# privacy-scaling-explorations/zkevm-specs

Hardware: AMD Instinct MI355X
Metric: BN254 constraint-rows/sec (higher is better)
Workload: dtype u256 (BN254 Fr: 4xu64 canonical cells, u32-limb Montgomery); 1 GPU; EVM circuit, 2^18 execution steps per GPU, mixed-opcode synthetic trace (BASELINE configs[2]); RW table 816377 rows, bytecode table 43913 rows; steps_per_gpu=262144, rw_rows=816377, bytecode_rows=43913, witness_copies=3

## Files before the change

### zkevm_specs_amd/csrc/zkevm_hip.hip

```cpp
#include <hip/hip_runtime.h>
#include <hip/hip_ext.h>
#include <stdio.h>
#include <string.h>
#include <stdlib.h>
#include <chrono>
#include <string>
#include <vector>

#include <atomic>
#include <mutex>
#include <dlfcn.h>

#include "../../include/zkevm_hip.h"
#include "kernels.hpp"
#include "dist_tally.hpp"
#include "host_index.hpp"
#include "code_dir_build.hpp"

#define ZK_MAX_DEVICES 64
#define ZK_ECDSA_CHUNK_LANES (1ull << 17)
static std::mutex g_dev_mutex;
static hipStream_t g_own_stream[ZK_MAX_DEVICES] = {nullptr};
static hipStream_t g_batch_stream[ZK_MAX_DEVICES][2] = {{nullptr}};
static hipStream_t g_side_stream[ZK_MAX_DEVICES] = {nullptr};
// ... 69 lines not shown
    return 0;
}
extern "C" void zk_shutdown(void) {
    arena_release_all();
    std::lock_guard<std::mutex> lock(g_dev_mutex);
    for (int d = 0; d < ZK_MAX_DEVICES; d++)
        if (g_own_stream[d]) {
            if (hipSetDevice(d) == hipSuccess) {
                (void)hipStreamDestroy(g_own_stream[d]);
                if (g_zero_row[d]) (void)hipFree(g_zero_row[d]);
                if (g_secp_comb[d]) (void)hipFree(g_secp_comb[d]);
                g_secp_comb[d] = nullptr;
            }
            for (int k = 0; k < 2; k++) {
                if (g_batch_stream[d][k]) (void)hipStreamDestroy(g_batch_stream[d][k]);
                g_batch_stream[d][k] = nullptr;
            }
            if (g_side_stream[d]) (void)hipStreamDestroy(g_side_stream[d]);
            g_side_stream[d] = nullptr;
            for (int k = 0; k < 4; k++) {
                if (g_block_stream[d][k]) (void)hipStreamDestroy(g_block_stream[d][k]);
                g_block_stream[d][k] = nullptr;
            }
            g_own_stream[d] = nullptr;
            g_zero_row[d] = nullptr;
        }
    t_stream = nullptr;
    t_device = -1;
}
extern "C" int zk_set_stream(void* st) {
    ARG_TRY(t_device >= 0, "zk_set_stream: call zk_init first");
    t_stream = st ? (hipStream_t)st : g_own_stream[t_device];
    return 0;
}
struct zk_session;
static int session_rebind_stream(zk_session* s, hipStream_t st);
extern "C" int zk_session_set_stream(zk_session* s, void* st) {
    ARG_TRY(s, "zk_session_set_stream: null session");
    return session_rebind_stream(s, (hipStream_t)st);
}

__global__ void tally_reset_kernel(ZkTally* t, u32* counter = nullptr) {
    t[threadIdx.x].fail_count = 0ull;
    t[threadIdx.x].first_fail = ~0ull;
    if (counter && threadIdx.x == 0) *counter = 0u;
}


__global__ void slots_fill_kernel(u32* slots, u32 n) {
    u32 i = blockIdx.x * blockDim.x + threadIdx.x;
    if (i < n) slots[i] = ZK_EMPTY_SLOT;
}

template <u64 (*HASH)(const ZkTable&, u32)>
__global__ void index_build_kernel(ZkTable t, u32* slots, const ZkRwMeta* unless_dense = nullptr) {
    u32 r = blockIdx.x * blockDim.x + threadIdx.x;
    if (r >= t.n || (unless_dense && unless_dense->dense)) return;
    u32 s = (u32)HASH(t, r) & t.mask;
    while (atomicCAS(&slots[s], ZK_EMPTY_SLOT, r) != ZK_EMPTY_SLOT) s = (s + 1) & t.mask;
}
__global__ void slots_fill_unless_dense_kernel(u32* slots, u32 n, const ZkRwMeta* unless_dense) {
    u32 i = blockIdx.x * blockDim.x + threadIdx.x;
    if (i < n && !unless_dense->dense) slots[i] = ZK_EMPTY_SLOT;
}
__global__ void mpt_index_build_kernel(ZkTable t, u32* slots) {
    u32 r = blockIdx.x * blockDim.x + threadIdx.x;
    if (r >= t.n) return;
    const u64 h = state_mpt_key_hash(t, r);
    u32 s = (u32)h & t.mask;
    const u32 v = state_mpt_slot_value(t, r, h);
    while (atomicCAS(&slots[s], ZK_EMPTY_SLOT, v) != ZK_EMPTY_SLOT) s = (s + 1) & t.mask;
}
__global__ void rw_dense_check_kernel(ZkTable t, ZkRwMeta* meta) {
    const u32 r = blockIdx.x * blockDim.x + threadIdx.x;
    if (r >= t.n) return;
    const u64* p = t.cells + (u64)r * RW_NCELLS * 4;
    const u64* p0 = t.cells;
    const u64 base = p0[0];
    const bool ok = (p0[1] | p0[2] | p0[3]) == 0 && (p[1] | p[2] | p[3]) == 0 && p[0] == base + r && base + r >= base;
    if (r == 0) meta->base = base;
    if (!ok) atomicAnd(&meta->dense, 0u);
}

struct EvmSortArgs {
    const u64* steps;
    u32 n_pairs;
    u32* hist;
    u32* hist_next;
    u32* taken;
    uint16_t* bin16;
    u32* group_start;
    u32* perm;
    ZkTally* tally;
    u32* defer_count;
    u32* early_host;
    u32 early_seq;
};
#define EVM_EARLY_WORD 36u
__device__ __forceinline__ void evm_state_hist_body(u32 vblock, const u64* steps, u32 n_pairs, u32* hist, u32* taken, uint16_t* bin16, ZkTally* tally,
                                                    u32* defer_count) {
    __shared__ u32 local[EVM_N_BINS];
    if (vblock == 0) {
        if (threadIdx.x == 0 && defer_count) *defer_count = 0u;
        if (threadIdx.x == 0) {
            tally->fail_count = 0ull;
            tally->first_fail = ~0ull;
        }
        for (u32 k = threadIdx.x; k < EVM_N_BINS; k += blockDim.x) taken[k] = 0;
    }
    for (u32 k = threadIdx.x; k < EVM_N_BINS; k += blockDim.x) local[k] = 0;
    __syncthreads();
    u32 i = vblock * blockDim.x + threadIdx.x;
    if (i < n_pairs) {
        const u32 bin = evm_state_bin((u32)steps[((u64)i * STEP_NCELLS + S_STATE) * 4]);
        bin16[i] = (uint16_t)bin;
        atomicAdd(&local[bin], 1u);
    }
    __syncthreads();
    for (u32 k = threadIdx.x; k < EVM_N_BINS; k += blockDim.x)
        if (local[k]) atomicAdd(&hist[k], local[k]);
}
__global__ void evm_state_hist_kernel(const u64* steps, u32 n_pairs, u32* hist, u32* taken, uint16_t* bin16, ZkTally* tally, u32* defer_count) {
    evm_state_hist_body(blockIdx.x, steps, n_pairs, hist, taken, bin16, tally, defer_count);
}
__device__ __forceinline__ void evm_state_scatter_body(u32 vblock, const uint16_t* bin16, u32 n_pairs, const u32* hist, u32* hist_next,
                                                       u32* taken, u32* group_start, u32* perm, u32* early_host = nullptr, u32 early_seq = 0u) {
    __shared__ u32 sa[EVM_N_BINS], sb[EVM_N_BINS];
    __shared__ u32 local[EVM_N_BINS];
    __shared__ u32 base[EVM_N_BINS];
    __shared__ u32 gsh[EVM_N_GROUPS + 1];
    const u32 k = threadIdx.x;
    u32 c = 0, c_real = 0;
    if (k < EVM_N_BINS) {
        c_real = hist[k];
        c = k < (u32)EVM_GROUP_WARM * 128u ? ((c_real + 63u) & ~63u) : c_real;
        sa[k] = c;
        local[k] = 0;
        if (vblock == 0) hist_next[k] = 0;
    }
    __syncthreads();
    u32* src = sa;
    u32* dst = sb;
    for (u32 off = 1; off < EVM_N_BINS; off <<= 1) {
        if (k < EVM_N_BINS) dst[k] = src[k] + (k >= off ? src[k - off] : 0u);
        __syncthreads();
        u32* t = src; src = dst; dst = t;
    }
    u32 excl = 0;
    if (k < EVM_N_BINS) {
        excl = src[k] - c;
        if (vblock == 0) {
            if ((k & 127u) == 0) group_start[k >> 7] = gsh[k >> 7] = excl;
            if (k == EVM_N_BINS - 1) group_start[EVM_N_GROUPS] = gsh[EVM_N_GROUPS] = src[k];
            for (u32 j = c_real; j < c; j++) perm[excl + j] = EVM_NO_PAIR;
        }
    }
    const u32 i = vblock * blockDim.x + threadIdx.x;
    u32 bin = 0, rank = 0;
    if (i < n_pairs) {
        bin = bin16[i];
        rank = atomicAdd(&local[bin], 1u);
    }
    __syncthreads();
    if (vblock == 0 && k == 0 && early_host) {
        __hip_atomic_store(&early_host[EVM_EARLY_WORD], gsh[EVM_GROUP_WARM + 1] - gsh[EVM_GROUP_WARM], __ATOMIC_RELAXED, __HIP_MEMORY_SCOPE_SYSTEM);
        __hip_atomic_store(&early_host[EVM_EARLY_WORD + 1], gsh[EVM_GROUP_COLD + 1] - gsh[EVM_GROUP_COLD], __ATOMIC_RELAXED, __HIP_MEMORY_SCOPE_SYSTEM);
        __threadfence_system();
        __hip_atomic_store(&early_host[EVM_EARLY_WORD + 2], early_seq, __ATOMIC_RELEASE, __HIP_MEMORY_SCOPE_SYSTEM);
    }
    if (k < EVM_N_BINS && local[k]) base[k] = excl + atomicAdd(&taken[k], local[k]);
    __syncthreads();
    if (i < n_pairs) perm[base[bin] + rank] = i;
}
__global__ __launch_bounds__(1024) void evm_state_scatter_kernel(const uint16_t* bin16, u32 n_pairs, const u32* hist, u32* hist_next,
                                                                 u32* taken, u32* group_start, u32* perm) {
    evm_state_scatter_body(blockIdx.x, bin16, n_pairs, hist, hist_next, taken, group_start, perm);
}
__global__ __launch_bounds__(256) void evm_open_fill_kernel(uint4* ff, u64 n_ff, uint4* zero, u64 n_zero) {
    const u64 stride = (u64)gridDim.x * blockDim.x;
    const uint4 F = make_uint4(~0u, ~0u, ~0u, ~0u), Z = make_uint4(0u, 0u, 0u, 0u);
    for (u64 i = (u64)blockIdx.x * blockDim.x + threadIdx.x; i < n_ff; i += stride) ff[i] = F;
    for (u64 i = (u64)blockIdx.x * blockDim.x + threadIdx.x; i < n_zero; i += stride) zero[i] = Z;
}
__device__ __forceinline__ void rw_prepare_quad(const ZkTable& t, u64* keys, EvmDyn* dyn, u32 vthread) {
    const u32 r = vthread >> 2, q = vthread & 3u;
    const bool in = r < t.n;
    uint4 c0 = make_uint4(0, 0, 0, 0), c1 = c0, c2 = c0;
    u64 base = 0;
    u32 flags = 3u;
    if (in) {
        const uint4* p = reinterpret_cast<const uint4*>(t.cells + (u64)r * RW_NCELLS * 4) + q;
        c0 = p[0];
        c1 = p[4];
        c2 = p[8];
        if (q == 0) {
            base = t.cells[0];
            if (t.flags) flags = t.flags[r];
        }
    }
    bool fit, dense_ok;
    u64 w0 = 0, w1 = 0, w2 = 0, w3 = 0;
    const bool z0hi = (c0.y | c0.z | c0.w) == 0u, z1hi = (c1.y | c1.z | c1.w) == 0u, z2hi = (c2.y | c2.z | c2.w) == 0u;
    const bool z0 = z0hi && c0.x == 0u, z1 = z1hi && c1.x == 0u, z2 = z2hi && c2.x == 0u;
    if (q == 0) {
        const u64 rwc = (u64)c0.x | ((u64)c0.y << 32);
        dense_ok = (c0.z | c0.w) == 0u && rwc == base + r && base + r >= base;
        fit = z1hi && c1.x <= 255u;
        w0 = (u64)(c1.x & 0xffu) << 8 | ((u64)(flags & 3u) << 56) | (1ull << 63);
        w2 = (u64)c2.x | ((u64)c2.y << 32);
        w3 = (u64)c2.z | ((u64)c2.w << 32);
    } else if (q == 1) {
        dense_ok = z0;
        fit = z1 && z2hi;
        w0 = (u64)c2.x << 24;
    } else if (q == 2) {
        dense_ok = true;
        fit = z0hi && c0.x <= 255u && (c1.z | c1.w) == 0u && z2hi && c2.x <= 255u;
        w0 = (u64)(c0.x & 0xffu) | ((u64)(c2.x & 0xffu) << 16);
        w1 = (u64)c1.x | ((u64)c1.y << 32);
    } else {
        dense_ok = true;
        fit = z0 && z1 && z2;
    }
    const u32 qshift = threadIdx.x & 60u;
    const bool fits = ((__ballot(fit) >> qshift) & 0xfull) == 0xfull;
    const unsigned long long nd = __ballot(in && !dense_ok);
    if (nd != 0ull && (threadIdx.x & 63u) == 0) atomicOr(&dyn->rw_sparse, 1u);
    if (r == 0 && q == 0 && in) dyn->rw_base = base;
#pragma unroll
    for (int m = 1; m <= 2; m <<= 1) {
        w0 |= __shfl_xor(w0, m);
        w1 |= __shfl_xor(w1, m);
        w2 |= __shfl_xor(w2, m);
        w3 |= __shfl_xor(w3, m);
    }
    if (!fits) w0 = w1 = w2 = w3 = 0;
    if (in && q < 2) {
        const u64 a = q == 0 ? w0 : w2, b2 = q == 0 ? w1 : w3;
        reinterpret_cast<uint4*>(keys + (u64)r * 4)[q] = make_uint4((u32)a, (u32)(a >> 32), (u32)b2, (u32)(b2 >> 32));
    }
}
#define EVM_OPEN_TABLES 8
struct EvmOpenTables {
    ZkTable t[EVM_OPEN_TABLES];
    u32 block_start[EVM_OPEN_TABLES + 2];
    const u64* wds;
    u32 n_wds;
    EvmDyn* dyn;
    ZkTally* tally;
    ZkTable rw;
    u64* rw_keys;
    u32 dir_block0, rw_block0;
    DirBuild dir;
    const u64* steps;
    u32 n_steps;
    u32* step_recs;
    u32 rec_block0;
    EvmSortArgs sort;
    u32 hist_block0;
    u32 lat_period;
#ifdef ZK_DIAG_P1
    u32 diag_skip;
#endif
};
__device__ __forceinline__ void evm_open_small_tables(const EvmOpenTables& o, u32 block) {
    int k = 0;
#pragma unroll
    for (int j = 1; j <= EVM_OPEN_TABLES; j++) k += block >= o.block_start[j] ? 1 : 0;
    const u32 r = (block - o.block_start[k]) * blockDim.x + threadIdx.x;
    if (k == EVM_OPEN_TABLES) {
        const bool nz = r < o.n_wds && !fr_is_zero(fr_load(o.wds + ((u64)r * 4 + 3) * 4));
        const unsigned long long b = __ballot(nz);
        if (b && (threadIdx.x & 63u) == 0) atomicAdd(&o.dyn->agg_total_wds, (u32)__popcll(b));
        return;
    }
    const ZkTable& t = o.t[k];
    const bool in = r < t.n;
    if (k == 0) {
        bool caller = false, present = false, invalid = false, bad = false;
        if (in) {
            const Fr tag = zk_table_cell(t, r, 1), lo = zk_table_cell(t, r, 3), hi = zk_table_cell(t, r, 4);
            caller = fr_eq_u64(tag, 4);
            present = caller && !(fr_is_zero(lo) && fr_is_zero(hi));
            const bool inv_row = fr_eq_u64(tag, 10);
            bad = inv_row && t.flags && (t.flags[r] & 1u);
            invalid = inv_row && fr_eq_u64(lo, 1);
        }
        const unsigned long long bc = __ballot(caller), bp = __ballot(present), bi = __ballot(invalid), bb = __ballot(bad);
        if ((threadIdx.x & 63u) == 0) {
            if (bc) atomicAdd(&o.dyn->agg_max_txs, (u32)__popcll(bc));
            if (bp) atomicAdd(&o.dyn->agg_total_txs, (u32)__popcll(bp));
            if (bi) atomicAdd(&o.dyn->agg_invalid_txs, (u32)__popcll(bi));
            if (bb) atomicOr(&o.dyn->agg_bad_invalid_rows, 1u);
        }
    }
    if (!in) return;
    u64 h;
    switch (k) {
    case 0: h = tx_key_hash(t, r); break;
    case 1: h = blk_key_hash(t, r); break;
    case 2: h = bc_key_hash(t, r); break;
    case 3: h = copy_key_hash(t, r); break;
    case 4: h = keccak_key_hash(t, r); break;
    case 5: h = expt_key_hash(t, r); break;
    case 6: h = sig_key_hash(t, r); break;
    default: h = ecc_key_hash(t, r); break;
    }
    u32* slots = const_cast<u32*>(t.slots);
    u32 s = (u32)h & t.mask;
    while (atomicCAS(&slots[s], ZK_EMPTY_SLOT, r) != ZK_EMPTY_SLOT) s = (s + 1) & t.mask;
}
__global__ __launch_bounds__(256) void evm_open_phase1_kernel(EvmOpenTables o) {
    if (blockIdx.x == 0 && threadIdx.x < 2) {
        o.tally[threadIdx.x].fail_count = 0ull;
        o.tally[threadIdx.x].first_fail = ~0ull;
    }
    u32 b = blockIdx.x;
    if (o.lat_period > 1u && b < o.rec_block0) {
        const u32 q = b / o.lat_period;
        b = (b == q * o.lat_period && q < o.rw_block0) ? q : o.rw_block0 + b - (q + 1u < o.rw_block0 ? q + 1u : o.rw_block0);
    }
#ifdef ZK_DIAG_P1
    {
        const u32 range = b < o.dir_block0 ? 1u : b < o.hist_block0 ? 2u : b < o.rw_block0 ? 4u : b < o.rec_block0 ? 8u : 16u;
        if (o.diag_skip & range) return;
    }
#endif
    if (b < o.dir_block0) evm_open_small_tables(o, b);
    else if (b < o.hist_block0) dirb_events_row(o.dir, (b - o.dir_block0) * blockDim.x + threadIdx.x);
    else if (b < o.rw_block0) evm_state_hist_body(b - o.hist_block0, o.sort.steps, o.sort.n_pairs, o.sort.hist, o.sort.taken, o.sort.bin16, o.sort.tally, o.sort.defer_count);
    else if (b < o.rec_block0) rw_prepare_quad(o.rw, o.rw_keys, o.dyn, (b - o.rw_block0) * blockDim.x + threadIdx.x);
    else evm_step_record_quad(o.steps, o.n_steps, o.step_recs, (b - o.rec_block0) * blockDim.x + threadIdx.x);
}
#define EVM_OPEN_RW_GENERIC_BLOCKS 64u
#define EVM_OPEN_P2_BLOCK 1024u
__global__ __launch_bounds__(1024) void evm_open_phase2_kernel(EvmOpenTables o, u32 scatter_blocks, u32 dir_blocks, u32 force_generic) {
    if (blockIdx.x < scatter_blocks) {
        evm_state_scatter_body(blockIdx.x, o.sort.bin16, o.sort.n_pairs, o.sort.hist, o.sort.hist_next, o.sort.taken, o.sort.group_start, o.sort.perm,
                               o.sort.early_host, o.sort.early_seq);
        return;
    }
    const u32 b = blockIdx.x - scatter_blocks;
    if (b < dir_blocks) {
        dirb_finalize_entry(o.dir, b * blockDim.x + threadIdx.x);
        return;
    }
    if (!force_generic && o.dyn->rw_sparse == 0u) return;
    if (force_generic && b == dir_blocks && threadIdx.x == 0) o.dyn->rw_sparse = 1u;
    u32* slots = const_cast<u32*>(o.rw.slots);
    const u32 stride = (gridDim.x - scatter_blocks - dir_blocks) * blockDim.x;
    for (u32 r = (b - dir_blocks) * blockDim.x + threadIdx.x; r < o.rw.n; r += stride) {
        u32 s = (u32)rw_key_hash(o.rw, r) & o.rw.mask;
        while (atomicCAS(&slots[s], ZK_EMPTY_SLOT, r) != ZK_EMPTY_SLOT) s = (s + 1) & o.rw.mask;
    }
}

__global__ void fr_op_kernel(int op, const u64* a, const u64* b, u64* out, u64 n) {
    u64 i = (u64)blockIdx.x * blockDim.x + threadIdx.x;
    if (i >= n) return;
    Fr x = fr_load(a + 4 * i), y = fr_load(b + 4 * i), r;
    switch (op) {
    case 0: r = fr_add(x, y); break;
    case 1: r = fr_sub(x, y); break;
    case 2: r = fr_mul(x, y); break;
    case 3: r = fr_mont(x, y); break;
    case 4: r = fr_neg(x); break;
    case 5: r = fr_inv(x); break;
    case 6: r = fr_div(x, y); break;
    case 16: r = sp_mul_p(x, y); break;
    case 17: r = sp_sqr_p(x); break;
    case 18: r = ecc_fq_mul_hook(x, y); break;
    case 26: r = sp_sqrt_p(x); break;
    case 27: r = sp_inv_p(x); break;
    default: r = fr_zero();
    }
    for (int k = 0; k < 4; k++) out[4 * i + k] = (u64)r.v[2 * k] | ((u64)r.v[2 * k + 1] << 32);
}

__global__ __launch_bounds__(64) void evm_publish_kernel(const u32* d, u32* h, u32 seq) {
    const u32 i = threadIdx.x;
    if (i < 32u) __hip_atomic_store(&h[i], d[i], __ATOMIC_RELAXED, __HIP_MEMORY_SCOPE_SYSTEM);
    __threadfence_system();
    if (i == 0u) __hip_atomic_store(&h[32], seq, __ATOMIC_RELEASE, __HIP_MEMORY_SCOPE_SYSTEM);
}
struct EvmResultBlock {
    EvmDyn dyn;
    u32 n_deferred_twin;
    u32 pad0[(64 - sizeof(EvmDyn)) / 4 - 1];
    ZkTally tally[2];
    u32 group_start[EVM_N_GROUPS + 1];
    u32 pad1[8 - (EVM_N_GROUPS + 1)];
};
static_assert(sizeof(EvmDyn) <= 64 && sizeof(EvmResultBlock) == 128, "EvmResultBlock layout");
enum SessionKind { SESSION_EXA = 17, SESSION_TXA = 16, SESSION_WITHDRAWAL = 15, SESSION_REKEY = 14, SESSION_PICOPY = 13, SESSION_PI = 12, SESSION_CPA = 11, SESSION_STATE = 1, SESSION_EVM = 2, SESSION_BYTECODE = 3, SESSION_EXP = 4, SESSION_COPY = 5, SESSION_SIGN = 6, SESSION_KECCAK = 7, SESSION_ASSIGN = 8, SESSION_ECDSA = 9, SESSION_BCA = 10 };

struct zk_session {
    SessionKind kind;
    int device = t_device;
    hipStream_t stream = t_stream;
    u64 n = 0;
    u64 eval_lo = 0, eval_hi = 0;
    std::vector<void*> owned;
    std::vector<int> owned_class;
    ZkTally* d_tally = nullptr;
    u32* d_status = nullptr;
    bool status_external = false;
    std::vector<hipEvent_t> ev;
    u32 launches = 0;
    u32 tally_pass = 0;
    ZkTally* tally_last = nullptr;
    StateArgs state;
    EvmArgs evm;
    BytecodeArgs bytecode;
    ExpArgs exp;
    CopyArgs copy;
    SignArgs sign;
    KeccakGenArgs keccak_gen;
    AssignArgs assign;
    EcdsaArgs ecdsa;
    BcaArgs bca;
    CpaArgs cpa;
    PiArgs pi;
    PiCopyArgs picopy;
    WithdrawalArgs withdrawal;
    TxAssignArgs txa;
    ExaArgs exa;
    u64 exa_n_table = 0;
    RekeyArgs rekey;
    RwkPlan rekey_plan_host;
    bool assign_from_rw = false;
    bool fused_order_ready = false;
    bool fused_verify = false;
    u32* rekey_status = nullptr;
// ... 285 lines not shown
    const u32 n = s->evm.n_pairs;
    u32* h_cur = (s->evm_pass & 1u) ? s->d_hist2 : s->d_hist;
    u32* h_next = (s->evm_pass & 1u) ? s->d_hist : s->d_hist2;
    s->evm_pass++;
    hipLaunchKernelGGL(evm_state_hist_kernel, dim3((n + ZK_HIST_BLOCK - 1) / ZK_HIST_BLOCK), dim3(ZK_HIST_BLOCK), 0, s->stream, s->evm.steps, n, h_cur, s->d_cursor, s->d_bin16, s->d_tally, s->evm.defer_count);
    hipLaunchKernelGGL(evm_state_scatter_kernel, dim3((n + 1023) / 1024), dim3(1024), 0, s->stream, s->d_bin16, n, h_cur, h_next, s->d_cursor,
                       s->d_group_start, s->d_perm);
    HIP_TRY(hipGetLastError());
    return 0;
}

static inline u32 index_cap(u64 n) {
    u32 cap = 16;
    while (cap < 2 * n + 2) cap <<= 1;
    return cap;
}

extern "C" int zk_evm_open(const zk_evm_tables* t, uint32_t opts, zk_session** out) {
    ARG_TRY(t_device >= 0, "zk_evm_open: call zk_init first");
    HIP_TRY(hipSetDevice(t_device));
    ARG_TRY(t && out && t->steps && t->n_steps >= 2 && t->n_steps < (1ull << 32), "zk_evm_open: bad arguments");
    ARG_TRY(t->n_rw < (1ull << 31) && t->n_bytecode < (1ull << 31) && t->n_tx < (1ull << 31) && t->n_block < (1ull << 31) &&
            t->n_copy < (1ull << 31) && t->n_keccak < (1ull << 31) && t->n_exp < (1ull << 31) && t->n_withdrawals < (1ull << 31) &&
            t->n_sig < (1ull << 31) && t->n_ecc < (1ull << 31),
            "zk_evm_open: table too large");
    ARG_TRY(t->aux_cells == 0 || (t->aux_cells >= 2 && t->aux_cells <= 64), "zk_evm_open: aux_cells must be 0 (= 2) or 2..64");
    const bool dev = opts & ZK_OPT_DEVICE_PTRS;
    const bool generic = opts & ZK_OPT_GENERIC_INDEX;
    zk_session* s = new zk_session();
    s->kind = SESSION_EVM;
    s->n = t->n_steps - 1;
    s->side_stream = (opts & ZK_OPT_SIDE_STREAM) != 0;
    int rc = 0;
    const void* p = nullptr;
    EvmArgs& E = s->evm;
    if ((rc = stage(s, t->steps, (size_t)t->n_steps * STEP_NCELLS * 32, dev, &p))) goto fail;
    E.steps = (const u64*)p;
    E.n_steps = t->n_steps;
    E.n_pairs = (u32)(t->n_steps - 1);
    if ((rc = table_stage(s, E.rw, t->rw, t->rw_flags, t->n_rw, RW_NCELLS, dev))) goto fail;
    if ((rc = table_stage(s, E.bytecode, t->bytecode, nullptr, t->n_bytecode, BYTECODE_NCELLS, dev))) goto fail;
    if ((rc = table_stage(s, E.tx, t->tx, t->tx_flags, t->n_tx, TX_NCELLS, dev))) goto fail;
    if ((rc = table_stage(s, E.block, t->block, t->block_flags, t->n_block, BLOCK_NCELLS, dev))) goto fail;
    if ((rc = table_stage(s, E.copy, t->copy, nullptr, t->n_copy, COPY_T_NCELLS, dev))) goto fail;
    if ((rc = table_stage(s, E.keccak, t->keccak, nullptr, t->n_keccak, KECCAK_NCELLS, dev))) goto fail;
    if ((rc = table_stage(s, E.exp, t->exp, nullptr, t->n_exp, EXP_T_NCELLS, dev))) goto fail;
    if ((rc = table_stage(s, E.sig, t->sig, nullptr, t->n_sig, SIG_T_NCELLS, dev))) goto fail;
    if ((rc = table_stage(s, E.ecc, t->ecc, nullptr, t->n_ecc, ECC_T_NCELLS, dev))) goto fail;
    if ((rc = table_stage(s, E.withdrawals, t->withdrawals, nullptr, t->n_withdrawals, 4, dev))) goto fail;
    E.withdrawals.slots = nullptr;
    E.withdrawals.mask = 0;
    E.aux = nullptr;
    E.aux_kind = nullptr;
    E.aux_cells = t->aux_cells ? t->aux_cells : 2u;
    if (t->aux && t->aux_kind) {
        if ((rc = stage(s, t->aux, (size_t)t->n_steps * E.aux_cells * 32, dev, &p))) goto fail;
        E.aux = (const u64*)p;
        if ((rc = stage(s, t->aux_kind, (size_t)t->n_steps * 4, dev, &p))) goto fail;
        E.aux_kind = (const u32*)p;
    }
    {
        ZkTable* const small[EVM_OPEN_TABLES] = {&E.tx, &E.block, &E.bytecode, &E.copy, &E.keccak, &E.exp, &E.sig, &E.ecc};
        const bool want_dir = !generic && t->n_bytecode != 0;
        size_t n_ff = 0;
        u32 caps[EVM_OPEN_TABLES];
        for (int k = 0; k < EVM_OPEN_TABLES; k++) { caps[k] = index_cap(small[k]->n); n_ff += caps[k]; }
        const u32 cap_rw = index_cap(E.rw.n), cap_big = want_dir ? index_cap(t->n_bytecode) : 0u;
        n_ff += (size_t)cap_rw + 2 * (size_t)cap_big + (want_dir ? DIRB_SMALL_SLOTS : 0u);
        u32* ff = nullptr;
        if ((rc = dev_alloc(s, (void**)&ff, n_ff * sizeof(u32)))) goto fail;
        u32* cur = ff;
        for (int k = 0; k < EVM_OPEN_TABLES; k++) { small[k]->slots = cur; small[k]->mask = caps[k] - 1; cur += caps[k]; }
        E.rw.slots = cur; E.rw.mask = cap_rw - 1; cur += cap_rw;
        u32* const dir_rep = cur; cur += cap_big;
        u32* const dir_first = cur; cur += cap_big;
        u32* const small_slots = cur;
        const size_t dyn_bytes = 256, hist_bytes = EVM_N_BINS * sizeof(u32), status_bytes = (((size_t)s->n * sizeof(u32)) + 15) & ~(size_t)15;
        const size_t zero_bytes = dyn_bytes + 2 * hist_bytes + status_bytes + 3 * (size_t)cap_big * 4;
        char* zero = nullptr;
        if ((rc = dev_alloc(s, (void**)&zero, zero_bytes))) goto fail;
        EvmResultBlock* const rb = (EvmResultBlock*)zero;
        EvmDyn* dyn = &rb->dyn;
        s->d_result = rb;
        if ((rc = arena_pinned(s->device, &s->h_result))) goto fail;
        {
            void* hd = nullptr;
            if (hipHostGetDevicePointer(&hd, s->h_result, 0) == hipSuccess) s->h_result_dev = (u32*)hd;
            (void)hipGetLastError();
        }
        static_assert(sizeof(EvmResultBlock) <= 256, "the result block outgrew its slot");
        static_assert((EVM_N_BINS * sizeof(u32)) % 16 == 0, "zero region pieces are 16-byte multiples");
        s->d_hist = (u32*)(zero + dyn_bytes);
        s->d_hist2 = (u32*)(zero + dyn_bytes + hist_bytes);
        s->d_status = (u32*)(zero + dyn_bytes + 2 * hist_bytes);
        u32* const dir_last = (u32*)(zero + dyn_bytes + 2 * hist_bytes + status_bytes);
        E.dyn = dyn;
        E.defer_count = &dyn->n_deferred;
        if ((rc = dev_alloc(s, (void**)&E.defer_list, (size_t)E.n_pairs * sizeof(u32)))) goto fail;
        s->d_tally = rb->tally;
        s->tally_last = s->d_tally;
        {
            const u64 n16 = n_ff / 4 + zero_bytes / 16;
            const u32 fill_grid = (u32)(n16 / 256 < 2048 ? (n16 + 255) / 256 : 2048);
            if (arena_event(s->device, &s->ev_open0) || arena_event(s->device, &s->ev_open1)) s->ev_open0 = s->ev_open1 = nullptr;
            hipExtLaunchKernelGGL(evm_open_fill_kernel, dim3(fill_grid ? fill_grid : 1u), dim3(256), 0, s->stream, s->ev_open0, nullptr, 0, (uint4*)ff,
                                  (u64)(n_ff / 4), (uint4*)zero, (u64)(zero_bytes / 16));
        }
        E.rw_dense = 0;
        E.rw_base = 0;
        E.rw_keys = nullptr;
        E.codes.n = 0;
        E.codes.mask = 0;
        E.codes.packed = nullptr;
        E.codes.entries = nullptr;
        E.codes.slots = nullptr;
        E.agg_max_txs = E.agg_total_txs = E.agg_invalid_txs = E.agg_bad_invalid_rows = E.agg_total_wds = 0;
        EvmOpenTables o;
        memset(&o, 0, sizeof o);
        u32 blk = 0;
        for (int k = 0; k < EVM_OPEN_TABLES; k++) { o.t[k] = *small[k]; o.block_start[k] = blk; blk += (small[k]->n + 255u) / 256u; }
        o.block_start[EVM_OPEN_TABLES] = blk;
        blk += (u32)((t->n_withdrawals + 255) / 256);
        o.block_start[EVM_OPEN_TABLES + 1] = blk;
        o.wds = E.withdrawals.cells;
        o.n_wds = (u32)t->n_withdrawals;
        o.dyn = dyn;
        o.tally = s->d_tally;
        o.rw = E.rw;
        if (t->n_rw && !generic) {
            u64* d_keys = nullptr;
            if ((rc = dev_alloc(s, (void**)&d_keys, (size_t)t->n_rw * 32))) goto fail;
            E.rw_keys = d_keys;
            o.rw_keys = d_keys;
        }
        const u32 rw_row_blocks = o.rw_keys ? (u32)((t->n_rw + 63) / 64) : 0u;
        o.dir_block0 = blk;
        u32 dir_row_blocks = 0;
        if (want_dir) {
            DirBuild& d = o.dir;
            d.rows = E.bytecode.cells;
            d.n = (u32)t->n_bytecode;
            d.rep = dir_rep;
            d.first = dir_first;
            d.last = dir_last;
            d.runs = dir_last + cap_big;
            d.bad = dir_last + 2 * (size_t)cap_big;
            d.big_mask = cap_big - 1;
            d.small_slots = small_slots;
            d.dyn = dyn;
            if ((rc = dev_alloc(s, (void**)&d.packed, (size_t)d.n * sizeof(uint16_t)))) goto fail;
            if ((rc = dev_alloc(s, (void**)&d.entries, (size_t)DIRB_MAX_ENTRIES * sizeof(ZkCodeEntry)))) goto fail;
            if ((rc = dev_alloc(s, (void**)&d.list, (size_t)DIRB_MAX_ENTRIES * 4))) goto fail;
            dir_row_blocks = (d.n + 255u) / 256u;
            E.codes.entries = d.entries;
            E.codes.slots = d.small_slots;
            E.codes.packed = d.packed;
        }
        if ((rc = dev_alloc(s, (void**)&s->d_cursor, EVM_N_BINS * sizeof(u32)))) goto fail;
        if ((rc = dev_alloc(s, (void**)&s->d_bin16, (size_t)E.n_pairs * sizeof(uint16_t)))) goto fail;
        s->d_group_start = rb->group_start;
        if ((rc = dev_alloc(s, (void**)&s->d_perm, ((size_t)E.n_pairs + EVM_PERM_PAD + 2 * EVM_HOT_BLOCK) * sizeof(u32)))) goto fail;
        const bool sorted = !(opts & ZK_OPT_NO_STATE_SORT);
        o.hist_block0 = o.dir_block0 + dir_row_blocks;
        u32 hist_blocks = 0, scatter_blocks = 0;
        if (sorted) {
            o.sort.steps = E.steps; o.sort.n_pairs = E.n_pairs; o.sort.hist = s->d_hist; o.sort.hist_next = s->d_hist2;
            o.sort.taken = s->d_cursor; o.sort.bin16 = s->d_bin16; o.sort.group_start = s->d_group_start; o.sort.perm = s->d_perm;
            o.sort.tally = s->d_tally;
            o.sort.defer_count = E.defer_count;
            if ((opts & ZK_OPT_SINGLE_PASS) && s->h_result_dev && evm_lazy_tail_enabled() && !(opts & ZK_OPT_SIDE_STREAM)) {
                static std::atomic<u32> g_early_seq{0};
                u32 q = ++g_early_seq;
                if (!q) q = ++g_early_seq;
                __atomic_store_n(&((u32*)s->h_result)[EVM_EARLY_WORD + 2], 0u, __ATOMIC_RELEASE);
                s->early_seq = q;
                o.sort.early_host = s->h_result_dev;
                o.sort.early_seq = q;
            }
            hist_blocks = (E.n_pairs + 255u) / 256u;
            scatter_blocks = (E.n_pairs + EVM_OPEN_P2_BLOCK - 1u) / EVM_OPEN_P2_BLOCK;
            s->evm_pass = 1;
            s->perm_ready = true;
        }
        o.rw_block0 = o.hist_block0 + hist_blocks;
        o.rec_block0 = o.rw_block0 + rw_row_blocks;
        u32 rec_blocks = 0;
        E.step_recs = nullptr;
        if (!(opts & ZK_OPT_SINGLE_PASS)) {
            u32* recs = nullptr;
            if ((rc = dev_alloc(s, (void**)&recs, (size_t)t->n_steps * EVM_REC_WORDS * sizeof(u32)))) goto fail;
            o.steps = E.steps; o.n_steps = (u32)t->n_steps; o.step_recs = recs;
            E.step_recs = recs;
            rec_blocks = (u32)((t->n_steps + 63) / 64);
        }
        const u32 grid1 = o.rec_block0 + rec_blocks;
        {
            static const u32 spread = [] { const char* e = getenv("ZK_P1_LAT_SPREAD"); const int v = e ? atoi(e) : 2; return (u32)(v < 0 ? 0 : v); }();
            o.lat_period = (o.rw_block0 && spread) ? o.rec_block0 / (spread * o.rw_block0) : 0u;
        }
#ifdef ZK_DIAG_P1
        if (const char* e = getenv("ZK_DIAG_P1_SKIP")) o.diag_skip = (u32)atoi(e);
#endif
        {
            const u32 dir_blocks = want_dir ? DIRB_MAX_ENTRIES / EVM_OPEN_P2_BLOCK : 0u;
            const u32 rw_blocks = t->n_rw ? EVM_OPEN_RW_GENERIC_BLOCKS : 0u;
            bool phase2 = scatter_blocks + dir_blocks + rw_blocks != 0;
#ifdef ZK_DIAG_P1
            if (o.diag_skip) phase2 = false;
#endif
            hipExtLaunchKernelGGL(evm_open_phase1_kernel, dim3(grid1 ? grid1 : 1u), dim3(256), 0, s->stream, nullptr, phase2 ? nullptr : s->ev_open1, 0, o);
            if (phase2)
                hipExtLaunchKernelGGL(evm_open_phase2_kernel, dim3(scatter_blocks + dir_blocks + rw_blocks), dim3(EVM_OPEN_P2_BLOCK), 0, s->stream, nullptr,
                                      s->ev_open1, 0, o, scatter_blocks, dir_blocks, generic ? 1u : 0u);
        }
        if (hipGetLastError() != hipSuccess) { rc = -2; g_err = "zk_evm_open: a build kernel failed to launch"; goto fail; }
    }
    E.opts = (t->begin_with_first_step ? 1u : 0u) | (t->end_with_last_step ? 2u : 0u);
    E.prof = nullptr;
    if (getenv("ZK_EVM_PROF")) {
        if ((rc = dev_alloc(s, (void**)&E.prof, 1024 * 4 * 8 * sizeof(unsigned long long)))) goto fail;
        if (hipMemsetAsync(E.prof, 0, 1024 * 4 * 8 * sizeof(unsigned long long), s->stream) != hipSuccess) { rc = -2; goto fail; }
    }
    E.perm = (opts & ZK_OPT_NO_STATE_SORT) ? nullptr : s->d_perm;
    *out = s;
    return 0;
fail:
    zk_close(s);
    return rc;
}

static void session_timing(zk_session* s, double pass_ms, double* open_ms, double* span_ms);
static int evm_enqueue_tail(zk_session* s);
static bool evm_publish_enqueue(zk_session* s);
extern "C" int zk_evm_verify(const zk_evm_tables* t, uint32_t opts, uint32_t* status_out, zk_result* result) {
    ARG_TRY(result, "zk_evm_verify: result is null");
    zk_session* s = nullptr;
    const auto h0 = std::chrono::steady_clock::now();
    int rc = zk_evm_open(t, opts | ZK_OPT_SINGLE_PASS, &s);
    if (rc) return rc;
    const auto h1 = std::chrono::steady_clock::now();
    const bool dev = opts & ZK_OPT_DEVICE_PTRS;
    rc = zk_launch(s, (dev && status_out) ? status_out : nullptr);
    const auto h2 = std::chrono::steady_clock::now();
    if (!rc) rc = zk_collect(s, result);
    const auto h3 = std::chrono::steady_clock::now();
    if (!rc) {
        t_timing[1] = result->kernel_ms;
        session_timing(s, result->kernel_ms, &t_timing[0], &t_timing[2]);
        for (int k = 0; k < 3; k++) t_timing_sum[k] += t_timing[k];
        t_timing_count++;
    }
    if (!rc && status_out && !dev) rc = zk_read_status(s, status_out);
    zk_close(s);
    const auto h4 = std::chrono::steady_clock::now();
    t_host_phase[0] = std::chrono::duration<double, std::micro>(h1 - h0).count();
    t_host_phase[1] = std::chrono::duration<double, std::micro>(h2 - h1).count();
    t_host_phase[2] = std::chrono::duration<double, std::micro>(h3 - h2).count();
    t_host_phase[3] = std::chrono::duration<double, std::micro>(h4 - h3).count();
    return rc;
}

extern "C" int zk_evm_verify_batch(const zk_evm_tables* const* t, uint64_t n, uint32_t opts, zk_result* results) {
    ARG_TRY(t_device >= 0, "zk_evm_verify_batch: call zk_init first");
    ARG_TRY((t && results) || n == 0, "zk_evm_verify_batch: bad arguments");
    for (uint64_t i = 0; i < n; i++) ARG_TRY(t[i], "zk_evm_verify_batch: null witness");
    HIP_TRY(hipSetDevice(t_device));
    {
        std::lock_guard<std::mutex> lock(g_dev_mutex);
        for (int k = 0; k < 2; k++)
            if (!g_batch_stream[t_device][k]) HIP_TRY(hipStreamCreateWithFlags(&g_batch_stream[t_device][k], hipStreamNonBlocking));
    }
    const hipStream_t caller = t_stream;
    HIP_TRY(hipStreamSynchronize(caller));
    zk_session* pend[2] = {nullptr, nullptr};
    int rc = 0;
    for (uint64_t i = 0; i < n + 2 && !rc; i++) {
        const int slot = (int)(i & 1u);
        if (pend[slot]) {
            rc = zk_collect(pend[slot], &results[i - 2]);
            zk_close(pend[slot]);
            pend[slot] = nullptr;
        }
        if (!rc && i < n) {
            t_stream = g_batch_stream[t_device][slot];
            rc = zk_evm_open(t[i], opts | ZK_OPT_SINGLE_PASS, &pend[slot]);
            t_stream = caller;
            if (!rc) rc = zk_launch(pend[slot], nullptr);
        }
        zk_session* const o = pend[slot ^ 1];
        if (!rc && o && !o->publish_enqueued) {
            rc = evm_enqueue_tail(o);
            if (!rc) o->publish_enqueued = evm_publish_enqueue(o);
        }
    }
    for (int k = 0; k < 2; k++)
        if (pend[k]) zk_close(pend[k]);
// ... 2320 lines not shown
```

Measured before the change: 1.534 billion rows/s.

## Replace global-atomic state sort with tiled histogram/scatter folded into fill and phase1 kernels

The state-bin counting sort is restructured into per-tile histograms computed inside the fill kernel, interleaved with fill blocks, plus a per-tile prefix-sum and wave-ballot scatter run inside the phase1 kernel. This removes the separate hist/scatter stages, which relied on global atomics over many blocks, and moves the sort earlier so it overlaps other open work. The bytecode directory events are now computed per row within the bytecode table branch instead of in separate blocks, and phase2 uses 256-thread blocks with more rw generic blocks. Each scatter tile re-sums counts over all prior tiles, and correctness depends on the new ballot-based ranking being stable.

```diff
diff --git a/zkevm_specs_amd/csrc/zkevm_hip.hip b/zkevm_specs_amd/csrc/zkevm_hip.hip
--- a/zkevm_specs_amd/csrc/zkevm_hip.hip
+++ b/zkevm_specs_amd/csrc/zkevm_hip.hip
@@ -175,20 +175,6 @@
     if (!ok) atomicAnd(&meta->dense, 0u);
 }
 
-struct EvmSortArgs {
-    const u64* steps;
-    u32 n_pairs;
-    u32* hist;
-    u32* hist_next;
-    u32* taken;
-    uint16_t* bin16;
-    u32* group_start;
-    u32* perm;
-    ZkTally* tally;
-    u32* defer_count;
-    u32* early_host;
-    u32 early_seq;
-};
 #define EVM_EARLY_WORD 36u
 __device__ __forceinline__ void evm_state_hist_body(u32 vblock, const u64* steps, u32 n_pairs, u32* hist, u32* taken, uint16_t* bin16, ZkTally* tally,
                                                     u32* defer_count) {
@@ -217,11 +203,10 @@
     evm_state_hist_body(blockIdx.x, steps, n_pairs, hist, taken, bin16, tally, defer_count);
 }
 __device__ __forceinline__ void evm_state_scatter_body(u32 vblock, const uint16_t* bin16, u32 n_pairs, const u32* hist, u32* hist_next,
-                                                       u32* taken, u32* group_start, u32* perm, u32* early_host = nullptr, u32 early_seq = 0u) {
+                                                       u32* taken, u32* group_start, u32* perm) {
     __shared__ u32 sa[EVM_N_BINS], sb[EVM_N_BINS];
     __shared__ u32 local[EVM_N_BINS];
     __shared__ u32 base[EVM_N_BINS];
-    __shared__ u32 gsh[EVM_N_GROUPS + 1];
     const u32 k = threadIdx.x;
     u32 c = 0, c_real = 0;
     if (k < EVM_N_BINS) {
@@ -243,8 +228,8 @@
     if (k < EVM_N_BINS) {
         excl = src[k] - c;
         if (vblock == 0) {
-            if ((k & 127u) == 0) group_start[k >> 7] = gsh[k >> 7] = excl;
-            if (k == EVM_N_BINS - 1) group_start[EVM_N_GROUPS] = gsh[EVM_N_GROUPS] = src[k];
+            if ((k & 127u) == 0) group_start[k >> 7] = excl;
+            if (k == EVM_N_BINS - 1) group_start[EVM_N_GROUPS] = src[k];
             for (u32 j = c_real; j < c; j++) perm[excl + j] = EVM_NO_PAIR;
         }
     }
@@ -255,12 +240,6 @@
         rank = atomicAdd(&local[bin], 1u);
     }
     __syncthreads();
-    if (vblock == 0 && k == 0 && early_host) {
-        __hip_atomic_store(&early_host[EVM_EARLY_WORD], gsh[EVM_GROUP_WARM + 1] - gsh[EVM_GROUP_WARM], __ATOMIC_RELAXED, __HIP_MEMORY_SCOPE_SYSTEM);
-        __hip_atomic_store(&early_host[EVM_EARLY_WORD + 1], gsh[EVM_GROUP_COLD + 1] - gsh[EVM_GROUP_COLD], __ATOMIC_RELAXED, __HIP_MEMORY_SCOPE_SYSTEM);
-        __threadfence_system();
-        __hip_atomic_store(&early_host[EVM_EARLY_WORD + 2], early_seq, __ATOMIC_RELEASE, __HIP_MEMORY_SCOPE_SYSTEM);
-    }
     if (k < EVM_N_BINS && local[k]) base[k] = excl + atomicAdd(&taken[k], local[k]);
     __syncthreads();
     if (i < n_pairs) perm[base[bin] + rank] = i;
@@ -269,11 +248,172 @@
                                                                  u32* taken, u32* group_start, u32* perm) {
     evm_state_scatter_body(blockIdx.x, bin16, n_pairs, hist, hist_next, taken, group_start, perm);
 }
-__global__ __launch_bounds__(256) void evm_open_fill_kernel(uint4* ff, u64 n_ff, uint4* zero, u64 n_zero) {
-    const u64 stride = (u64)gridDim.x * blockDim.x;
+#define EVM_SORT_TILE_MIN 4096u
+#define EVM_SORT_MAX_TILES 256u
+#define EVM_SORT_BLOCK 256u
+static inline u32 evm_sort_tile(u32 n_pairs) {
+    u64 t = EVM_SORT_TILE_MIN;
+    while (t * EVM_SORT_MAX_TILES < n_pairs) t <<= 1;
+    return (u32)t;
+}
+struct EvmSortArgs {
+    const u64* steps;
+    u32 n_pairs;
+    u32 tile, n_tiles;
+    u32* tile_counts;
+    uint16_t* bin16;
+    u32* group_start;
+    u32* perm;
+    u32* early_host;
+    u32 early_seq;
+};
+__device__ __forceinline__ void evm_tile_hist_body(u32 tile_idx, const EvmSortArgs& a) {
+    __shared__ u32 local[EVM_N_BINS];
+    for (u32 k = threadIdx.x; k < EVM_N_BINS; k += EVM_SORT_BLOCK) local[k] = 0;
+    __syncthreads();
+    const u64 lo = (u64)tile_idx * a.tile;
+    const u64 hi = lo + a.tile < (u64)a.n_pairs ? lo + a.tile : (u64)a.n_pairs;
+    for (u64 i0 = lo + threadIdx.x; i0 < hi; i0 += 8u * EVM_SORT_BLOCK) {
+        u32 st[8];
+#pragma unroll
+        for (u32 j = 0; j < 8; j++) {
+            const u64 i = i0 + j * EVM_SORT_BLOCK;
+            st[j] = i < hi ? (u32)a.steps[(i * STEP_NCELLS + S_STATE) * 4] : 0u;
+        }
+#pragma unroll
+        for (u32 j = 0; j < 8; j++) {
+            const u64 i = i0 + j * EVM_SORT_BLOCK;
+            if (i < hi) {
+                const u32 bin = evm_state_bin(st[j]);
+                a.bin16[i] = (uint16_t)bin;
+                atomicAdd(&local[bin], 1u);
+            }
+        }
+    }
+    __syncthreads();
+    for (u32 k = threadIdx.x; k < EVM_N_BINS; k += EVM_SORT_BLOCK) a.tile_counts[(u64)tile_idx * EVM_N_BINS + k] = local[k];
+}
+__device__ __forceinline__ void evm_tile_scatter_body(u32 tile_idx, const EvmSortArgs& a) {
+    constexpr u32 PER = (EVM_N_BINS + EVM_SORT_BLOCK - 1) / EVM_SORT_BLOCK, WAVES = EVM_SORT_BLOCK / 64u;
+    __shared__ u32 s_start[EVM_N_BINS];
+    __shared__ u32 s_scan[2][EVM_SORT_BLOCK];
+    __shared__ u32 s_cur[WAVES][EVM_N_BINS];
+    const u32 k = threadIdx.x, w = k >> 6, lane = k & 63u;
+    for (u32 j = k; j < WAVES * EVM_N_BINS; j += EVM_SORT_BLOCK) (&s_cur[0][0])[j] = 0;
+    __syncthreads();
+    const u64 lo = (u64)tile_idx * a.tile;
+    const u64 hi = lo + a.tile < (u64)a.n_pairs ? lo + a.tile : (u64)a.n_pairs;
+    const u32 quarter = a.tile / WAVES;
+    const u64 wlo = lo + (u64)w * quarter < hi ? lo + (u64)w * quarter : hi;
+    const u64 whi = wlo + quarter < hi ? wlo + quarter : hi;
+    for (u64 i = wlo + lane; i < whi; i += 64u) atomicAdd(&s_cur[w][a.bin16[i]], 1u);
+    u32 tot[PER], pre[PER];
+#pragma unroll
+    for (u32 q = 0; q < PER; q++) {
+        const u32 b = k + q * EVM_SORT_BLOCK;
+        u32 p = 0, t_all = 0;
+        if (b < EVM_N_BINS) {
+            for (u32 t = 0; t < tile_idx; t++) p += a.tile_counts[(u64)t * EVM_N_BINS + b];
+            t_all = p;
+            for (u32 t = tile_idx; t < a.n_tiles; t++) t_all += a.tile_counts[(u64)t * EVM_N_BINS + b];
+            s_start[b] = b < (u32)EVM_GROUP_WARM * 128u ? ((t_all + 63u) & ~63u) : t_all;
+        }
+        pre[q] = p;
+        tot[q] = t_all;
+    }
+    __syncthreads();
+    u32 mine[PER], sum = 0;
+#pragma unroll
+    for (u32 q = 0; q < PER; q++) {
+        const u32 b = k * PER + q;
+        mine[q] = b < EVM_N_BINS ? s_start[b] : 0u;
+        sum += mine[q];
+    }
+    s_scan[0][k] = sum;
+    __syncthreads();
+    u32 cur = 0;
+    for (u32 off = 1; off < EVM_SORT_BLOCK; off <<= 1) {
+        s_scan[cur ^ 1u][k] = s_scan[cur][k] + (k >= off ? s_scan[cur][k - off] : 0u);
+        __syncthreads();
+        cur ^= 1u;
+    }
+    {
+        u32 run = s_scan[cur][k] - sum;
+#pragma unroll
+        for (u32 q = 0; q < PER; q++) {
+            const u32 b = k * PER + q;
+            if (b < EVM_N_BINS) s_start[b] = run;
+            run += mine[q];
+        }
+    }
+    const u32 total = s_scan[cur][EVM_SORT_BLOCK - 1u];
+    __syncthreads();
+#pragma unroll
+    for (u32 q = 0; q < PER; q++) {
+        const u32 b = k + q * EVM_SORT_BLOCK;
+        if (b < EVM_N_BINS) {
+            const u32 start = s_start[b];
+            if (tile_idx == 0 && b < (u32)EVM_GROUP_WARM * 128u)
+                for (u32 j = start + tot[q]; j < start + ((tot[q] + 63u) & ~63u); j++) a.perm[j] = EVM_NO_PAIR;
+            u32 run = start + pre[q];
+#pragma unroll
+            for (u32 v = 0; v < WAVES; v++) {
+                const u32 c = s_cur[v][b];
+                s_cur[v][b] = run;
+                run += c;
+            }
+        }
+    }
+    if (tile_idx == 0) {
+        if (k < (u32)EVM_N_GROUPS) a.group_start[k] = s_start[k * 128u];
+        if (k == (u32)EVM_N_GROUPS) a.group_start[k] = total;
+        if (k == 0 && a.early_host) {
+            const u32 warm0 = s_start[EVM_GROUP_WARM * 128u], cold0 = s_start[EVM_GROUP_COLD * 128u];
+            __hip_atomic_store(&a.early_host[EVM_EARLY_WORD], cold0 - warm0, __ATOMIC_RELAXED, __HIP_MEMORY_SCOPE_SYSTEM);
+            __hip_atomic_store(&a.early_host[EVM_EARLY_WORD + 1], total - cold0, __ATOMIC_RELAXED, __HIP_MEMORY_SCOPE_SYSTEM);
+            __threadfence_system();
+            __hip_atomic_store(&a.early_host[EVM_EARLY_WORD + 2], a.early_seq, __ATOMIC_RELEASE, __HIP_MEMORY_SCOPE_SYSTEM);
+        }
+    }
+    __syncthreads();
+    volatile u32* const cursor = s_cur[w];
+    for (u64 i0 = wlo; i0 < whi; i0 += 64u) {
+        const u64 i = i0 + lane;
+        const bool in = i < whi;
+        const u32 bin = in ? (u32)a.bin16[i] : 0u;
+        unsigned long long same = __ballot(in);
+#pragma unroll
+        for (u32 bit = 0; bit < 10u; bit++) {
+            const bool one = (bin >> bit) & 1u;
+            const unsigned long long m = __ballot(one);
+            same &= one ? m : ~m;
+        }
+        if (in) {
+            const u32 rank = (u32)__popcll(same & ((1ull << lane) - 1ull));
+            const u32 at = cursor[bin];
+            __builtin_amdgcn_wave_barrier();
+            if (rank == 0) cursor[bin] = at + (u32)__popcll(same);
+            a.perm[at + rank] = (u32)i;
+        }
+        __builtin_amdgcn_wave_barrier();
+    }
+}
+static_assert(EVM_N_BINS <= 1024, "evm_tile_scatter_body matches bins by 10 ballots");
+__global__ __launch_bounds__(256) void evm_open_fill_kernel(uint4* ff, u64 n_ff, uint4* zero, u64 n_zero, EvmSortArgs sort, u32 tile_period) {
+    u32 b = blockIdx.x, fill_blocks = gridDim.x;
+    if (sort.perm) {
+        fill_blocks -= sort.n_tiles;
+        const u32 q = b / tile_period;
+        if (b == q * tile_period && q < sort.n_tiles) {
+            evm_tile_hist_body(q, sort);
+            return;
+        }
+        b -= q + 1u < sort.n_tiles ? q + 1u : sort.n_tiles;
+    }
+    const u64 stride = (u64)fill_blocks * blockDim.x;
     const uint4 F = make_uint4(~0u, ~0u, ~0u, ~0u), Z = make_uint4(0u, 0u, 0u, 0u);
-    for (u64 i = (u64)blockIdx.x * blockDim.x + threadIdx.x; i < n_ff; i += stride) ff[i] = F;
-    for (u64 i = (u64)blockIdx.x * blockDim.x + threadIdx.x; i < n_zero; i += stride) zero[i] = Z;
+    for (u64 i = (u64)b * blockDim.x + threadIdx.x; i < n_ff; i += stride) ff[i] = F;
+    for (u64 i = (u64)b * blockDim.x + threadIdx.x; i < n_zero; i += stride) zero[i] = Z;
 }
 __device__ __forceinline__ void rw_prepare_quad(const ZkTable& t, u64* keys, EvmDyn* dyn, u32 vthread) {
     const u32 r = vthread >> 2, q = vthread & 3u;
@@ -350,7 +490,7 @@
     u32* step_recs;
     u32 rec_block0;
     EvmSortArgs sort;
-    u32 hist_block0;
+    u32 sort_block0;
     u32 lat_period;
 #ifdef ZK_DIAG_P1
     u32 diag_skip;
@@ -369,6 +509,9 @@
     }
     const ZkTable& t = o.t[k];
     const bool in = r < t.n;
+#ifndef ZK_TMP_BC_TWO_READS
+    if (k == 2 && o.dir.n) dirb_events_row(o.dir, r);
+#endif
     if (k == 0) {
         bool caller = false, present = false, invalid = false, bad = false;
         if (in) {
@@ -413,27 +556,28 @@
         const u32 q = b / o.lat_period;
         b = (b == q * o.lat_period && q < o.rw_block0) ? q : o.rw_block0 + b - (q + 1u < o.rw_block0 ? q + 1u : o.rw_block0);
     }
+    if (b < o.rw_block0) {
+        const u32 n_sort = o.rw_block0 - o.sort_block0;
+        b = b < n_sort ? o.sort_block0 + b : b - n_sort;
+    }
 #ifdef ZK_DIAG_P1
     {
-        const u32 range = b < o.dir_block0 ? 1u : b < o.hist_block0 ? 2u : b < o.rw_block0 ? 4u : b < o.rec_block0 ? 8u : 16u;
+        const u32 range = b < o.dir_block0 ? 1u : b < o.sort_block0 ? 2u : b < o.rw_block0 ? 4u : b < o.rec_block0 ? 8u : 16u;
         if (o.diag_skip & range) return;
     }
 #endif
     if (b < o.dir_block0) evm_open_small_tables(o, b);
-    else if (b < o.hist_block0) dirb_events_row(o.dir, (b - o.dir_block0) * blockDim.x + threadIdx.x);
-    else if (b < o.rw_block0) evm_state_hist_body(b - o.hist_block0, o.sort.steps, o.sort.n_pairs, o.sort.hist, o.sort.taken, o.sort.bin16, o.sort.tally, o.sort.defer_count);
+#ifdef ZK_TMP_BC_TWO_READS
+    else if (b < o.sort_block0) dirb_events_row(o.dir, (b - o.dir_block0) * blockDim.x + threadIdx.x);
+#endif
+    else if (b < o.rw_block0) evm_tile_scatter_body(b - o.sort_block0, o.sort);
     else if (b < o.rec_block0) rw_prepare_quad(o.rw, o.rw_keys, o.dyn, (b - o.rw_block0) * blockDim.x + threadIdx.x);
     else evm_step_record_quad(o.steps, o.n_steps, o.step_recs, (b - o.rec_block0) * blockDim.x + threadIdx.x);
 }
-#define EVM_OPEN_RW_GENERIC_BLOCKS 64u
-#define EVM_OPEN_P2_BLOCK 1024u
-__global__ __launch_bounds__(1024) void evm_open_phase2_kernel(EvmOpenTables o, u32 scatter_blocks, u32 dir_blocks, u32 force_generic) {
-    if (blockIdx.x < scatter_blocks) {
-        evm_state_scatter_body(blockIdx.x, o.sort.bin16, o.sort.n_pairs, o.sort.hist, o.sort.hist_next, o.sort.taken, o.sort.group_start, o.sort.perm,
-                               o.sort.early_host, o.sort.early_seq);
-        return;
-    }
-    const u32 b = blockIdx.x - scatter_blocks;
+#define EVM_OPEN_P2_BLOCK 256u
+#define EVM_OPEN_RW_GENERIC_BLOCKS 256u
+__global__ __launch_bounds__(256) void evm_open_phase2_kernel(EvmOpenTables o, u32 dir_blocks, u32 force_generic) {
+    const u32 b = blockIdx.x;
     if (b < dir_blocks) {
         dirb_finalize_entry(o.dir, b * blockDim.x + threadIdx.x);
         return;
@@ -441,7 +585,7 @@
     if (!force_generic && o.dyn->rw_sparse == 0u) return;
     if (force_generic && b == dir_blocks && threadIdx.x == 0) o.dyn->rw_sparse = 1u;
     u32* slots = const_cast<u32*>(o.rw.slots);
-    const u32 stride = (gridDim.x - scatter_blocks - dir_blocks) * blockDim.x;
+    const u32 stride = (gridDim.x - dir_blocks) * blockDim.x;
     for (u32 r = (b - dir_blocks) * blockDim.x + threadIdx.x; r < o.rw.n; r += stride) {
         u32 s = (u32)rw_key_hash(o.rw, r) & o.rw.mask;
         while (atomicCAS(&slots[s], ZK_EMPTY_SLOT, r) != ZK_EMPTY_SLOT) s = (s + 1) & o.rw.mask;
@@ -893,12 +1037,6 @@
         EvmResultBlock* const rb = (EvmResultBlock*)zero;
         EvmDyn* dyn = &rb->dyn;
         s->d_result = rb;
-        if ((rc = arena_pinned(s->device, &s->h_result))) goto fail;
-        {
-            void* hd = nullptr;
-            if (hipHostGetDevicePointer(&hd, s->h_result, 0) == hipSuccess) s->h_result_dev = (u32*)hd;
-            (void)hipGetLastError();
-        }
         static_assert(sizeof(EvmResultBlock) <= 256, "the result block outgrew its slot");
         static_assert((EVM_N_BINS * sizeof(u32)) % 16 == 0, "zero region pieces are 16-byte multiples");
         s->d_hist = (u32*)(zero + dyn_bytes);
@@ -907,16 +1045,38 @@
         u32* const dir_last = (u32*)(zero + dyn_bytes + 2 * hist_bytes + status_bytes);
         E.dyn = dyn;
         E.defer_count = &dyn->n_deferred;
-        if ((rc = dev_alloc(s, (void**)&E.defer_list, (size_t)E.n_pairs * sizeof(u32)))) goto fail;
         s->d_tally = rb->tally;
         s->tally_last = s->d_tally;
+        const bool sorted = !(opts & ZK_OPT_NO_STATE_SORT);
+        EvmSortArgs sort;
+        memset(&sort, 0, sizeof sort);
+        s->d_group_start = rb->group_start;
+        if ((rc = dev_alloc(s, (void**)&s->d_bin16, (size_t)E.n_pairs * sizeof(uint16_t)))) goto fail;
+        if ((rc = dev_alloc(s, (void**)&s->d_perm, ((size_t)E.n_pairs + EVM_PERM_PAD + 2 * EVM_HOT_BLOCK) * sizeof(u32)))) goto fail;
+        if (sorted) {
+            sort.steps = E.steps; sort.n_pairs = E.n_pairs;
+            sort.tile = evm_sort_tile(E.n_pairs);
+            sort.n_tiles = (u32)(((u64)E.n_pairs + sort.tile - 1) / sort.tile);
+            if ((rc = dev_alloc(s, (void**)&sort.tile_counts, (size_t)sort.n_tiles * EVM_N_BINS * sizeof(u32)))) goto fail;
+            sort.bin16 = s->d_bin16; sort.group_start = s->d_group_start; sort.perm = s->d_perm;
+        }
         {
             const u64 n16 = n_ff / 4 + zero_bytes / 16;
-            const u32 fill_grid = (u32)(n16 / 256 < 2048 ? (n16 + 255) / 256 : 2048);
-            if (arena_event(s->device, &s->ev_open0) || arena_event(s->device, &s->ev_open1)) s->ev_open0 = s->ev_open1 = nullptr;
-            hipExtLaunchKernelGGL(evm_open_fill_kernel, dim3(fill_grid ? fill_grid : 1u), dim3(256), 0, s->stream, s->ev_open0, nullptr, 0, (uint4*)ff,
-                                  (u64)(n_ff / 4), (uint4*)zero, (u64)(zero_bytes / 16));
-        }
+            const u32 fill_grid = (u32)(n16 / 256 < 2048 ? (n16 + 255) / 256 : 2048), fill_blocks = fill_grid ? fill_grid : 1u;
+            const u32 grid0 = fill_blocks + sort.n_tiles;
+            const u32 tile_period = sort.n_tiles && grid0 / (2u * sort.n_tiles) > 1u ? grid0 / (2u * sort.n_tiles) : 1u;
+            if (arena_event(s->device, &s->ev_open0)) s->ev_open0 = nullptr;
+            hipExtLaunchKernelGGL(evm_open_fill_kernel, dim3(grid0), dim3(256), 0, s->stream, s->ev_open0, nullptr, 0, (uint4*)ff,
+                                  (u64)(n_ff / 4), (uint4*)zero, (u64)(zero_bytes / 16), sort, tile_period);
+        }
+        if (arena_event(s->device, &s->ev_open1)) s->ev_open1 = nullptr;
+        if ((rc = arena_pinned(s->device, &s->h_result))) goto fail;
+        {
+            void* hd = nullptr;
+            if (hipHostGetDevicePointer(&hd, s->h_result, 0) == hipSuccess) s->h_result_dev = (u32*)hd;
+            (void)hipGetLastError();
+        }
+        if ((rc = dev_alloc(s, (void**)&E.defer_list, (size_t)E.n_pairs * sizeof(u32)))) goto fail;
         E.rw_dense = 0;
         E.rw_base = 0;
         E.rw_keys = nullptr;
@@ -962,23 +1122,18 @@
             if ((rc = dev_alloc(s, (void**)&d.packed, (size_t)d.n * sizeof(uint16_t)))) goto fail;
             if ((rc = dev_alloc(s, (void**)&d.entries, (size_t)DIRB_MAX_ENTRIES * sizeof(ZkCodeEntry)))) goto fail;
             if ((rc = dev_alloc(s, (void**)&d.list, (size_t)DIRB_MAX_ENTRIES * 4))) goto fail;
+#ifdef ZK_TMP_BC_TWO_READS
             dir_row_blocks = (d.n + 255u) / 256u;
+#endif
             E.codes.entries = d.entries;
             E.codes.slots = d.small_slots;
             E.codes.packed = d.packed;
         }
         if ((rc = dev_alloc(s, (void**)&s->d_cursor, EVM_N_BINS * sizeof(u32)))) goto fail;
-        if ((rc = dev_alloc(s, (void**)&s->d_bin16, (size_t)E.n_pairs * sizeof(uint16_t)))) goto fail;
-        s->d_group_start = rb->group_start;
-        if ((rc = dev_alloc(s, (void**)&s->d_perm, ((size_t)E.n_pairs + EVM_PERM_PAD + 2 * EVM_HOT_BLOCK) * sizeof(u32)))) goto fail;
-        const bool sorted = !(opts & ZK_OPT_NO_STATE_SORT);
-        o.hist_block0 = o.dir_block0 + dir_row_blocks;
-        u32 hist_blocks = 0, scatter_blocks = 0;
+        o.sort_block0 = o.dir_block0 + dir_row_blocks;
+        u32 sort_blocks = 0;
         if (sorted) {
-            o.sort.steps = E.steps; o.sort.n_pairs = E.n_pairs; o.sort.hist = s->d_hist; o.sort.hist_next = s->d_hist2;
-            o.sort.taken = s->d_cursor; o.sort.bin16 = s->d_bin16; o.sort.group_start = s->d_group_start; o.sort.perm = s->d_perm;
-            o.sort.tally = s->d_tally;
-            o.sort.defer_count = E.defer_count;
+            o.sort = sort;
             if ((opts & ZK_OPT_SINGLE_PASS) && s->h_result_dev && evm_lazy_tail_enabled() && !(opts & ZK_OPT_SIDE_STREAM)) {
                 static std::atomic<u32> g_early_seq{0};
                 u32 q = ++g_early_seq;
@@ -988,12 +1143,10 @@
                 o.sort.early_host = s->h_result_dev;
                 o.sort.early_seq = q;
             }
-            hist_blocks = (E.n_pairs + 255u) / 256u;
-            scatter_blocks = (E.n_pairs + EVM_OPEN_P2_BLOCK - 1u) / EVM_OPEN_P2_BLOCK;
-            s->evm_pass = 1;
+            sort_blocks = sort.n_tiles;
             s->perm_ready = true;
         }
-        o.rw_block0 = o.hist_block0 + hist_blocks;
+        o.rw_block0 = o.sort_block0 + sort_blocks;
         o.rec_block0 = o.rw_block0 + rw_row_blocks;
         u32 rec_blocks = 0;
         E.step_recs = nullptr;
@@ -1015,14 +1168,14 @@
         {
             const u32 dir_blocks = want_dir ? DIRB_MAX_ENTRIES / EVM_OPEN_P2_BLOCK : 0u;
             const u32 rw_blocks = t->n_rw ? EVM_OPEN_RW_GENERIC_BLOCKS : 0u;
-            bool phase2 = scatter_blocks + dir_blocks + rw_blocks != 0;
+            bool phase2 = dir_blocks + rw_blocks != 0;
 #ifdef ZK_DIAG_P1
             if (o.diag_skip) phase2 = false;
 #endif
             hipExtLaunchKernelGGL(evm_open_phase1_kernel, dim3(grid1 ? grid1 : 1u), dim3(256), 0, s->stream, nullptr, phase2 ? nullptr : s->ev_open1, 0, o);
             if (phase2)
-                hipExtLaunchKernelGGL(evm_open_phase2_kernel, dim3(scatter_blocks + dir_blocks + rw_blocks), dim3(EVM_OPEN_P2_BLOCK), 0, s->stream, nullptr,
-                                      s->ev_open1, 0, o, scatter_blocks, dir_blocks, generic ? 1u : 0u);
+                hipExtLaunchKernelGGL(evm_open_phase2_kernel, dim3(dir_blocks + rw_blocks), dim3(EVM_OPEN_P2_BLOCK), 0, s->stream, nullptr,
+                                      s->ev_open1, 0, o, dir_blocks, generic ? 1u : 0u);
         }
         if (hipGetLastError() != hipSuccess) { rc = -2; g_err = "zk_evm_open: a build kernel failed to launch"; goto fail; }
     }
```

Measured after the change: 1.096 billion rows/s. 28.5% lower.
